# zouyuoz/SVS-UNet-PyTorch

Hardware: AMD Instinct MI355X
Metric: spectrogram-tiles/sec (512x128) U-Net fwd+bwd (L1 train step incl. Adam) (higher is better)
Workload: dtype f32; 1 GPU; train.py L1-loss step, 512x128 tiles, batch 64 per GPU; global_batch=64, parallelism=dp1, mode=train

## Files before the change

### svs_unet_pytorch_amd/csrc/gemm_wgrad.hip

```cpp
#include <stdlib.h>

#include "internal.h"
#include "mfma_split.h"

struct WgradArgs {
  const float* s; long lds; int Hs, Ws, Cs;
  const float* l; long ldl; int Hl, Wl, Cl;
  int B;
  float* slab;
  long pix_per_split;
  int ws_shift, hs_shift;
  int b_shift;
};

template <int T> __device__ __forceinline__ void load_vec(const float* p, float (&f)[T]);
template <> __device__ __forceinline__ void load_vec<4>(const float* p, float (&f)[4]) {
  const f32x4 v = *(const f32x4*)p; f[0] = v[0]; f[1] = v[1]; f[2] = v[2]; f[3] = v[3];
}
template <> __device__ __forceinline__ void load_vec<2>(const float* p, float (&f)[2]) {
  const float2 v = *(const float2*)p; f[0] = v.x; f[1] = v.y;
}
template <int T> __device__ __forceinline__ void store_vec(float* p, const float (&f)[T]);
template <> __device__ __forceinline__ void store_vec<4>(float* p, const float (&f)[4]) { *(f32x4*)p = (f32x4){f[0], f[1], f[2], f[3]}; }
template <> __device__ __forceinline__ void store_vec<2>(float* p, const float (&f)[2]) { *(float2*)p = make_float2(f[0], f[1]); }

template <int BM, int BN, int WM, int WN, bool SKIP = false, bool SPLIT = false, int PF = 1>
__global__ __launch_bounds__(256) void wgrad_gemm_kernel(WgradArgs p) {
  constexpr int TM = BM / WM / 16;
  constexpr int TN = BN / WN / 16;
  constexpr int LDA = BM + 4, LDB = BN + 4;
  constexpr int CA = BM / 4, CB = BN / 4;
  constexpr int RA = (16 * CA + 255) / 256, RB = (16 * CB + 255) / 256;
  static_assert(WM * WN == 4, "4 waves");

  __shared__ __attribute__((aligned(16))) float As[2][16 * LDA];
  __shared__ __attribute__((aligned(16))) float Bs[2][16 * LDB];

  const int t = threadIdx.x;
  const int lane = t & 63, wave = t >> 6;
  const int wm = wave / WN, wn = wave % WN;
  const int lrow = lane & 15, q = lane >> 4;

  const int Ntot = 25 * p.Cl;
  const int cs0 = blockIdx.x * BM;
  const int n0 = blockIdx.y * BN;
  const long P = (long)p.B * p.Hs * p.Ws;
  const long p_begin = (long)blockIdx.z * p.pix_per_split;
  long p_end = p_begin + p.pix_per_split;
  if (p_end > P) p_end = P;

  constexpr unsigned OOB = 0x80000000u;
  int ak[RA], ac[RA]; bool aok[RA];
#pragma unroll
  for (int r = 0; r < RA; ++r) {
    const int idx = t + 256 * r;
    ak[r] = idx / CA; ac[r] = idx % CA; aok[r] = idx < 16 * CA;
  }
  int bk[RB], bc[RB], bkh[RB], bkw[RB], bcl[RB]; bool bok[RB];
#pragma unroll
  for (int r = 0; r < RB; ++r) {
    const int idx = t + 256 * r;
    bk[r] = idx / CB; bc[r] = idx % CB;
    const int n = n0 + bc[r] * 4;
    bok[r] = (idx < 16 * CB) && (n < Ntot);
    const int tap = bok[r] ? n / p.Cl : 0;
    bcl[r] = bok[r] ? n - tap * p.Cl : 0;
    bkh[r] = tap / 5; bkw[r] = tap - bkh[r] * 5;
  }

  int bj[RB], bi[RB]; unsigned bimg[RB];
#pragma unroll
  for (int r = 0; r < RB; ++r) {
    const unsigned pix = (unsigned)(p_begin + bk[r]);
    const unsigned row = pix / (unsigned)p.Ws;
    bj[r] = (int)(pix - row * (unsigned)p.Ws);
    const unsigned img = row / (unsigned)p.Hs;
    bi[r] = (int)(row - img * (unsigned)p.Hs);
    bimg[r] = img * (unsigned)(p.Hl * p.Wl);
  }
  const unsigned img_stride = (unsigned)(p.Hl * p.Wl);
  auto advance = [&]() {
#pragma unroll
    for (int r = 0; r < RB; ++r) {
      unsigned j = (unsigned)bj[r] + 16u, i = (unsigned)bi[r];
      if (p.ws_shift >= 0) { i += j >> p.ws_shift; j &= (unsigned)p.Ws - 1u; }
      else { const unsigned q = j / (unsigned)p.Ws; j -= q * (unsigned)p.Ws; i += q; }
      unsigned nb;
      if (p.hs_shift >= 0) { nb = i >> p.hs_shift; i &= (unsigned)p.Hs - 1u; }
      else { nb = i / (unsigned)p.Hs; i -= nb * (unsigned)p.Hs; }
      bj[r] = (int)j; bi[r] = (int)i; bimg[r] += nb * img_stride;
    }
  };

  unsigned a_voff[RA];
#pragma unroll
  for (int r = 0; r < RA; ++r) a_voff[r] = aok[r] ? (unsigned)(((long)ak[r] * p.lds + cs0 + ac[r] * 4) * 4) : OOB;
  const __amdgpu_buffer_rsrc_t rs = __builtin_amdgcn_make_buffer_rsrc((void*)(p.s + p_begin * p.lds), 0, OOB, 0x00020000);
  const __amdgpu_buffer_rsrc_t rl = __builtin_amdgcn_make_buffer_rsrc((void*)p.l, 0, OOB, 0x00020000);
  const int HsWs = p.Hs * p.Ws, HlWl = p.Hl * p.Wl;
  unsigned a_voff_s[RA], b_voff_s[RB];
  int tap_lo = 0, tap_hi = 0;
  if (SKIP) {
#pragma unroll
    for (int r = 0; r < RA; ++r) a_voff_s[r] = aok[r] ? (unsigned)((((long)ak[r] * HsWs) * p.lds + cs0 + ac[r] * 4) * 4) : OOB;
#pragma unroll
    for (int r = 0; r < RB; ++r)
      b_voff_s[r] = (unsigned)((((long)bk[r] * HlWl + bkh[r] * p.Wl + bkw[r]) * p.ldl + bcl[r]) * 4);
    tap_lo = n0 / p.Cl;
    const int nlast = (n0 + BN - 1 < Ntot - 1) ? n0 + BN - 1 : Ntot - 1;
    tap_hi = nlast / p.Cl;
  }
  const __amdgpu_buffer_rsrc_t rs_all = __builtin_amdgcn_make_buffer_rsrc((void*)p.s, 0, OOB, 0x00020000);
  const __amdgpu_buffer_rsrc_t rl_sh = __builtin_amdgcn_make_buffer_rsrc((void*)(p.l - (2L * p.Wl + 2) * p.ldl), 0, OOB, 0x00020000);
  auto position = [&](int pk, int& i, int& j, int& b0) {
    const int pos = pk >> p.b_shift;
    b0 = pk & (p.B - 1);
    i = pos >> p.ws_shift;
    j = pos & (p.Ws - 1);
  };
  auto first_valid = [&](int pk) -> int {
    if (!SKIP) return pk;
    while (pk < (int)p_end) {
      int i, j, b0;
      position(pk, i, j, b0);
      bool any = false;
      for (int tp = tap_lo; tp <= tap_hi; ++tp) {
        const int kh = tp / 5, kw = tp - kh * 5;
        any = any || ((unsigned)(2 * i - 2 + kh) < (unsigned)p.Hl && (unsigned)(2 * j - 2 + kw) < (unsigned)p.Wl);
      }
      if (any) return pk;
      pk = ((pk >> p.b_shift) + 1) << p.b_shift;
    }
    return (int)p_end;
  };
  f32x4 ra[RA], rb[RB];
  f32x4 ra2[PF == 2 ? RA : 1], rb2[PF == 2 ? RB : 1];
  auto load_tile_skip = [&](int pk, f32x4 (&ra)[RA], f32x4 (&rb)[RB]) __attribute__((always_inline)) {
    int i, j, b0;
    position(pk, i, j, b0);
    const int soff_a = __builtin_amdgcn_readfirstlane((int)((((long)b0 * HsWs + (i * p.Ws + j)) * p.lds) * 4));
    const int soff_b = __builtin_amdgcn_readfirstlane((int)((((long)b0 * HlWl + 2 * i * p.Wl + 2 * j) * p.ldl) * 4));
    const int left = (int)p_end - pk;
#pragma unroll
    for (int r = 0; r < RA; ++r) {
      const unsigned vo = ak[r] < left ? a_voff_s[r] : OOB;
      ra[r] = __builtin_bit_cast(f32x4, __builtin_amdgcn_raw_buffer_load_b128(rs_all, (int)vo, soff_a, 0));
    }
#pragma unroll
    for (int r = 0; r < RB; ++r) {
      const int ih = 2 * i - 2 + bkh[r], iw = 2 * j - 2 + bkw[r];
      const bool ok = bok[r] && bk[r] < left && (unsigned)ih < (unsigned)p.Hl && (unsigned)iw < (unsigned)p.Wl;
      rb[r] = __builtin_bit_cast(f32x4, __builtin_amdgcn_raw_buffer_load_b128(rl_sh, (int)(ok ? b_voff_s[r] : OOB), soff_b, 0));
    }
  };
  auto load_tile = [&](long pk, f32x4 (&ra)[RA], f32x4 (&rb)[RB]) __attribute__((always_inline)) {
    const int soff_a = (int)((pk - p_begin) * p.lds * 4);
    const int left = (int)(p_end - pk);
#pragma unroll
    for (int r = 0; r < RA; ++r) {
      const unsigned vo = ak[r] < left ? a_voff[r] : OOB;
      ra[r] = __builtin_bit_cast(f32x4, __builtin_amdgcn_raw_buffer_load_b128(rs, (int)vo, soff_a, 0));
    }
#pragma unroll
    for (int r = 0; r < RB; ++r) {
      const int ih = 2 * bi[r] - 2 + bkh[r], iw = 2 * bj[r] - 2 + bkw[r];
      const bool ok = bok[r] && bk[r] < left && (unsigned)ih < (unsigned)p.Hl && (unsigned)iw < (unsigned)p.Wl;
      const unsigned vo = ((bimg[r] + (unsigned)(ih * p.Wl + iw)) * (unsigned)p.ldl + (unsigned)bcl[r]) * 4u;
      rb[r] = __builtin_bit_cast(f32x4, __builtin_amdgcn_raw_buffer_load_b128(rl, (int)(ok ? vo : OOB), 0, 0));
    }
    advance();
  };
  auto store_tile = [&](int buf, const f32x4 (&ra)[RA], const f32x4 (&rb)[RB]) __attribute__((always_inline)) {
#pragma unroll
    for (int r = 0; r < RA; ++r)
      if (aok[r]) *(f32x4*)(&As[buf][ak[r] * LDA + ac[r] * 4]) = ra[r];
#pragma unroll
    for (int r = 0; r < RB; ++r)
      if (t + 256 * r < 16 * CB) *(f32x4*)(&Bs[buf][bk[r] * LDB + bc[r] * 4]) = rb[r];
  };

  f32x4 acc[TM][TN];
#pragma unroll
  for (int i = 0; i < TM; ++i)
// ... 36 lines not shown
  if constexpr (PF == 2) {
    int pk1 = first_valid(pk + 16);
    if (pk < (int)p_end) fetch(pk, ra, rb);
    if (pk1 < (int)p_end) fetch(pk1, ra2, rb2);
    if (pk < (int)p_end) store_tile(0, ra, rb);
    __syncthreads();
    while (pk < (int)p_end) {
      int pk2 = first_valid(pk1 + 16);
      if (pk2 < (int)p_end) fetch(pk2, ra, rb);
      multiply(0);
      if (pk1 < (int)p_end) store_tile(1, ra2, rb2);
      __syncthreads();
      pk = pk1; pk1 = pk2;
      if (pk >= (int)p_end) break;
      pk2 = first_valid(pk1 + 16);
      if (pk2 < (int)p_end) fetch(pk2, ra2, rb2);
      multiply(1);
      if (pk1 < (int)p_end) store_tile(0, ra, rb);
      __syncthreads();
      pk = pk1; pk1 = pk2;
    }
  } else {
    if (pk < (int)p_end) {
      fetch(pk, ra, rb);
      store_tile(0, ra, rb);
    }
    __syncthreads();
    for (int it = 0; pk < (int)p_end; ++it) {
      const int buf = it & 1;
      const int pkn = first_valid(pk + 16);
      const bool more = pkn < (int)p_end;
      if (more) fetch(pkn, ra, rb);
      pk = pkn;
      multiply(buf);
      if (more) store_tile(buf ^ 1, ra, rb);
      __syncthreads();
    }
  }

  float* slab = p.slab + (long)blockIdx.z * p.Cs * Ntot;
#pragma unroll
  for (int i = 0; i < TM; ++i)
#pragma unroll
    for (int r = 0; r < 4; ++r) {
      const int cs = cs0 + wm * (TM * 16) + TM * (4 * q + r) + i;
      const int n = n0 + wn * (TN * 16) + TN * lrow;
      if (n < Ntot) {
        float v[TN];
#pragma unroll
        for (int j = 0; j < TN; ++j) v[j] = acc[i][j][r];
        store_vec<TN>(&slab[(long)cs * Ntot + n], v);
      }
    }
}

struct WgWinArgs {
  const float* s; long lds; const float* l; long ldl;
  int B, Hs, Ws, Cs, Hl, Wl, Cl;
  float* slab;
  int ntiles, tiles_per_block;
};

template <int MT>
__global__ __launch_bounds__(256, 2) void wgrad_window_kernel(WgWinArgs p) {
  constexpr int TH = 4, TW = 16, KS = 4 / MT, CSB = 16 * MT;
  constexpr int LS = CSB + 16;
  constexpr int LH = 2 * TH + 3, LW = 2 * TW + 3, LL = 24;
  constexpr int NS = TH * TW * (CSB / 4), NL = LH * LW * 4;
  constexpr int RS = (NS + 255) / 256, RL = (NL + 255) / 256;
  constexpr int KSTEPS = TH * TW / 4 / KS;
  constexpr unsigned OOB = 0x80000000u;
  __shared__ __attribute__((aligned(16))) float Ssm[TH * TW * LS];
  __shared__ __attribute__((aligned(16))) float Lsm[LH * LW * LL];
  const int t = threadIdx.x, lane = t & 63, wave = t >> 6;
  const int lrow = lane & 15, q = lane >> 4;
  const int mt = wave % MT, half = wave / MT;
  const int mchunks = p.Cs / CSB;
  const int m0 = (blockIdx.y % mchunks) * CSB, cl0 = (blockIdx.y / mchunks) * 16;
  const int tiles_w = (p.Ws + TW - 1) / TW, tiles_h = (p.Hs + TH - 1) / TH;
  const int tile_lo = blockIdx.x * p.tiles_per_block;
  const int tile_hi = min(tile_lo + p.tiles_per_block, p.ntiles);

  f32x4 sreg[RS], lreg[RL];
  auto fetch = [&](int tile) {
    const int tw0 = (tile % tiles_w) * TW, th0 = ((tile / tiles_w) % tiles_h) * TH;
    const long b = tile / (tiles_w * tiles_h);
    const __amdgpu_buffer_rsrc_t rs = __builtin_amdgcn_make_buffer_rsrc((void*)(p.s + b * p.Hs * p.Ws * p.lds), 0, OOB, 0x00020000);
    const __amdgpu_buffer_rsrc_t rl = __builtin_amdgcn_make_buffer_rsrc((void*)(p.l + b * p.Hl * p.Wl * p.ldl), 0, OOB, 0x00020000);
#pragma unroll
    for (int r = 0; r < RS; ++r) {
      const int e = t + 256 * r;
      const int c4 = e % (CSB / 4), px = e / (CSB / 4);
      const int sh = th0 + px / TW, sw = tw0 + px % TW;
      const bool ok = e < NS && sh < p.Hs && sw < p.Ws;
      const unsigned vo = ok ? (unsigned)(((sh * p.Ws + sw) * (int)p.lds + m0 + c4 * 4) * 4) : OOB;
      sreg[r] = __builtin_bit_cast(f32x4, __builtin_amdgcn_raw_buffer_load_b128(rs, (int)vo, 0, 0));
    }
#pragma unroll
    for (int r = 0; r < RL; ++r) {
      const int e = t + 256 * r;
      const int c4 = e & 3, px = e >> 2;
      const int ih = 2 * th0 - 2 + px / LW, iw = 2 * tw0 - 2 + px % LW;
      const bool ok = e < NL && (unsigned)ih < (unsigned)p.Hl && (unsigned)iw < (unsigned)p.Wl;
      const unsigned vo = ok ? (unsigned)(((ih * p.Wl + iw) * (int)p.ldl + cl0 + c4 * 4) * 4) : OOB;
      lreg[r] = __builtin_bit_cast(f32x4, __builtin_amdgcn_raw_buffer_load_b128(rl, (int)vo, 0, 0));
    }
  };
  auto stage = [&]() {
#pragma unroll
    for (int r = 0; r < RS; ++r) {
      const int e = t + 256 * r;
      if (e < NS) *(f32x4*)(&Ssm[(e / (CSB / 4)) * LS + (e % (CSB / 4)) * 4]) = sreg[r];
    }
#pragma unroll
    for (int r = 0; r < RL; ++r) {
      const int e = t + 256 * r;
      if (e < NL) *(f32x4*)(&Lsm[(e >> 2) * LL + (e & 3) * 4]) = lreg[r];
    }
  };

  f32x4 acc[25];
#pragma unroll
  for (int i = 0; i < 25; ++i) acc[i] = (f32x4){0.f, 0.f, 0.f, 0.f};
  const float* abase = &Ssm[(half * (TH / KS) * TW + q) * LS + mt * 16 + lrow];
  const float* bbase = &Lsm[(half * (TH / KS) * 2 * LW + 2 * q) * LL + lrow];

  if (tile_lo < tile_hi) fetch(tile_lo);
  for (int tile = tile_lo; tile < tile_hi; ++tile) {
    __syncthreads();
    stage();
    __syncthreads();
    if (tile + 1 < tile_hi) fetch(tile + 1);
#pragma unroll
    for (int ks = 0; ks < KSTEPS; ++ks) {
      const int sh = ks / 4, sg = ks % 4;
      const float a = abase[(sh * TW + sg * 4) * LS];
#pragma unroll
      for (int tap = 0; tap < 25; ++tap) {
        const int kh = tap / 5, kw = tap % 5;
        const float bv = bbase[((2 * sh + kh) * LW + 8 * sg + kw) * LL];
        acc[tap] = __builtin_amdgcn_mfma_f32_16x16x4f32(a, bv, acc[tap], 0, 0, 0);
      }
    }
  }
  const int Ntot = 25 * p.Cl;
  float* slab = p.slab + ((long)blockIdx.x * KS + half) * p.Cs * Ntot;
#pragma unroll
  for (int tap = 0; tap < 25; ++tap)
#pragma unroll
    for (int r = 0; r < 4; ++r)
      slab[(long)(m0 + mt * 16 + 4 * q + r) * Ntot + tap * p.Cl + cl0 + lrow] = acc[tap][r];
}

__global__ __launch_bounds__(256) void wgrad_reduce_kernel(const float* __restrict__ slab, int ksplit, int Cs, int Cl,
                                                           float* __restrict__ dw) {
  __shared__ float tile[25][65];
  const int clt = Cl < 64 ? Cl : 64;
  const int cs = blockIdx.x, cl0 = blockIdx.y * clt;
  const long zstride = (long)Cs * Cl * 25;
  const float* src0 = slab + (long)cs * 25 * Cl + cl0;
  const int q4 = clt >> 2;
  for (int e = threadIdx.x; e < 25 * q4; e += 256) {
    const int tap = e / q4, cl = (e - tap * q4) * 4;
    const float* src = src0 + (long)tap * Cl + cl;
    f32x4 acc = {0.f, 0.f, 0.f, 0.f};
    int z = 0;
    for (; z + 4 <= ksplit; z += 4, src += 4 * zstride) {
      const f32x4 a = *(const f32x4*)src, b = *(const f32x4*)(src + zstride), c = *(const f32x4*)(src + 2 * zstride), d = *(const f32x4*)(src + 3 * zstride);
      acc += a; acc += b; acc += c; acc += d;
    }
    for (; z < ksplit; ++z, src += zstride) acc += *(const f32x4*)src;
    tile[tap][cl] = acc[0]; tile[tap][cl + 1] = acc[1]; tile[tap][cl + 2] = acc[2]; tile[tap][cl + 3] = acc[3];
  }
  __syncthreads();
  float* dst = dw + ((long)cs * Cl + cl0) * 25;
  for (int e = threadIdx.x; e < 25 * clt; e += 256) {
    const int cl = e / 25, tap = e - cl * 25;
    dst[e] = tile[tap][cl];
  }
}

struct WgradTile { int cfg, BM, BN, ksplit; long pps; };
static WgradTile plan_wgrad(int B, int Hs, int Ws, int Cs, int Cl) {
  WgradTile pl{};
  if (Cs % 128 == 0) { pl.cfg = 0; pl.BM = 128; }
  else if (Cs % 64 == 0) { pl.cfg = 1; pl.BM = 64; }
  else { pl.cfg = 2; pl.BM = 32; }
  if (pl.cfg == 0 && ((long)B * Hs * Ws <= 1024 || Cl <= 32)) { pl.cfg = 1; pl.BM = 64; }
  if (svs_tune_on(SVS_TUNE_WGRAD_CFG)) {
    const int c = (int)svs_tune(SVS_TUNE_WGRAD_CFG);
    if (c == 0 && Cs % 128 == 0) { pl.cfg = 0; pl.BM = 128; }
    if (c == 1 && Cs % 64 == 0) { pl.cfg = 1; pl.BM = 64; }
    if (c == 2 && Cs % 32 == 0) { pl.cfg = 2; pl.BM = 32; }
  }
  pl.BN = 128;
  const long P = (long)B * Hs * Ws;
  const long blocks_mn = (long)(Cs / pl.BM) * ((25L * Cl + pl.BN - 1) / pl.BN);
  long ks = (1024 + blocks_mn - 1) / blocks_mn;
  const long cap = P / 128 > 1 ? P / 128 : 1;
  if (ks > cap) ks = cap;
  if (ks > 512) ks = 512;
  if (ks < 1) ks = 1;
  if (svs_tune_on(SVS_TUNE_WGRAD_KSPLIT)) { long f = svs_tune(SVS_TUNE_WGRAD_KSPLIT); if (f >= 1 && f <= cap) ks = f; }
  long pps = (P + ks - 1) / ks;
  pps = (pps + 15) / 16 * 16;
  ks = (P + pps - 1) / pps;
  pl.ksplit = (int)ks;
  pl.pps = pps;
  return pl;
}

#define WG_GROUPS 8

struct WgWinPlan { int eligible, use, MT, gy, gx, tpb, ntiles, nslab; };
static WgWinPlan plan_wgrad_window(int B, int Hs, int Ws, int Cs, int Cl) {
  WgWinPlan w{};
  w.eligible = (Cl == 16 || Cl == 32) && (Cs == 32 || Cs == 64 || Cs == 128);
  w.ntiles = B * ((Hs + 3) / 4) * ((Ws + 15) / 16);
  w.use = w.eligible && w.ntiles >= 1024;
  if (svs_tune_on(SVS_TUNE_WGRAD_WINDOW)) { const int f = (int)svs_tune(SVS_TUNE_WGRAD_WINDOW); w.use = (f == 0) ? 0 : (f == 2) ? w.eligible : w.use; }
  if (!w.eligible) return w;
  w.MT = (Cs % 64 == 0) ? 4 : 2;
  w.gy = (Cs / (16 * w.MT)) * (Cl / 16);
  int gx = 512 / w.gy;
  if (gx > w.ntiles) gx = w.ntiles;
  w.tpb = (w.ntiles + gx - 1) / gx;
  w.gx = (w.ntiles + w.tpb - 1) / w.tpb;
  w.nslab = w.gx * (4 / w.MT);
  return w;
}

struct WgradPlan {
  WgWinPlan win;
  WgradTile tile;
  int WM, WN, pf;
  bool skip, split;
  dim3 grid;
  int nslab;
};
static WgradPlan plan_wgrad_call(int B, int Hs, int Ws, int Cs, int Cl, long lds, int Hl, int Wl, long ldl) {
  WgradPlan p{};
  p.win = plan_wgrad_window(B, Hs, Ws, Cs, Cl);
  p.win.use = p.win.use && (long)Hs * Ws * lds * 4 < (1L << 31) && (long)Hl * Wl * ldl * 4 < (1L << 31);
  if (p.win.use) {
    p.grid = dim3(p.win.gx, p.win.gy);
    p.nslab = p.win.nslab;
    return p;
  }
  p.tile = plan_wgrad(B, Hs, Ws, Cs, Cl);
  p.WM = p.tile.cfg == 0 ? 2 : 1;
  p.WN = 4 / p.WM;
  const bool can_skip = B >= 16 && (B & (B - 1)) == 0 && (Ws & (Ws - 1)) == 0 && (long)B * Hs * Ws * lds * 4 < (1L << 31);
  const long f = svs_tune(SVS_TUNE_WGRAD_SKIP);
  p.skip = f == 0 ? false : f == 2 ? can_skip : can_skip && Ws <= 8;
  p.pf = p.skip && p.tile.cfg <= 1 ? 2 : 1;
  p.split = svs_tune(SVS_TUNE_MFMA_SPLIT) > 0;
  p.grid = dim3((unsigned)(Cs / p.tile.BM), (unsigned)((25 * Cl + p.tile.BN - 1) / p.tile.BN), (unsigned)p.tile.ksplit);
  p.nslab = p.tile.ksplit;
  return p;
}

size_t svs_wgrad_gemm_workspace(int B, int Hs, int Ws, int Cs, int Cl) {
  const WgWinPlan w = plan_wgrad_window(B, Hs, Ws, Cs, Cl);
  int nslab = plan_wgrad(B, Hs, Ws, Cs, Cl).ksplit;
  if (w.eligible && w.nslab > nslab) nslab = w.nslab;
  return ((size_t)nslab + WG_GROUPS) * Cs * 25 * Cl * sizeof(float);
}

static int wgrad_reduce_run(const float* slabs, int nslab, int Cs, int Cl, float* dw, float* tmp, hipStream_t stream) {
  const long n = (long)Cs * 25 * Cl;
  if (nslab > 2 * WG_GROUPS) {
    const int per = (nslab + WG_GROUPS - 1) / WG_GROUPS;
    const int groups = (nslab + per - 1) / per;
    if (int rc = svs_reduce_slabs_run(slabs, nslab, per, groups, n, tmp, stream)) return rc;
    slabs = tmp;
    nslab = groups;
  }
  hipLaunchKernelGGL(wgrad_reduce_kernel, dim3((unsigned)Cs, (unsigned)((Cl + 63) / 64)), dim3(256), 0, stream, slabs, nslab, Cs,
                     Cl, dw);
  SVS_CHECK_LAUNCH("wgrad_reduce");
  return SVS_OK;
}

template <bool SPLIT, int BM, int WM, int WN>
static void launch_wgrad_tile(const WgradArgs& a, const WgradPlan& p, hipStream_t stream) {
  constexpr int PF2 = BM == 32 ? 1 : 2;
  if (!p.skip) hipLaunchKernelGGL((wgrad_gemm_kernel<BM, 128, WM, WN, false, SPLIT>), p.grid, dim3(256), 0, stream, a);
  else if (p.pf == 2) hipLaunchKernelGGL((wgrad_gemm_kernel<BM, 128, WM, WN, true, SPLIT, PF2>), p.grid, dim3(256), 0, stream, a);
  else hipLaunchKernelGGL((wgrad_gemm_kernel<BM, 128, WM, WN, true, SPLIT>), p.grid, dim3(256), 0, stream, a);
}
template <bool SPLIT>
static void launch_wgrad_gemm(const WgradArgs& a, const WgradPlan& p, hipStream_t stream) {
  switch (p.tile.cfg) {
    case 0: launch_wgrad_tile<SPLIT, 128, 2, 2>(a, p, stream); break;
    case 1: launch_wgrad_tile<SPLIT, 64, 1, 4>(a, p, stream); break;
    default: launch_wgrad_tile<SPLIT, 32, 1, 4>(a, p, stream); break;
  }
}

int svs_wgrad_gemm_run(const float* s, long lds, int B, int Hs, int Ws, int Cs, const float* l, long ldl, int Hl,
                       int Wl, int Cl, float* dw, void* ws, size_t ws_bytes, hipStream_t stream, const char* who) {
  SVS_REQUIRE(s && l && dw, "%s: null pointer", who);
  SVS_REQUIRE(Cs >= 32 && Cs % 32 == 0 && Cl >= 16 && Cl % 4 == 0, "%s: unsupported channels Cs=%d Cl=%d", who, Cs, Cl);
  SVS_REQUIRE(Hs == svs_conv_out(Hl) && Ws == svs_conv_out(Wl), "%s: small grid %dx%d does not match %dx%d", who, Hs, Ws, Hl, Wl);
  SVS_REQUIRE(lds >= Cs && lds % 4 == 0 && ldl >= Cl && ldl % 4 == 0, "%s: bad ld", who);
  SVS_REQUIRE(svs_aligned16(s) && svs_aligned16(l) && svs_aligned16(ws), "%s: pointers must be 16-byte aligned", who);
  const size_t need = svs_wgrad_gemm_workspace(B, Hs, Ws, Cs, Cl);
  if (!ws || ws_bytes < need) {
    svs_set_error("%s: workspace too small (%zu < %zu)", who, ws_bytes, need);
    return SVS_ERR_WORKSPACE;
  }
  const WgradPlan p = plan_wgrad_call(B, Hs, Ws, Cs, Cl, lds, Hl, Wl, ldl);
  if (p.win.use) {
    WgWinArgs wa{s, lds, l, ldl, B, Hs, Ws, Cs, Hl, Wl, Cl, (float*)ws, p.win.ntiles, p.win.tpb};
    if (p.win.MT == 4) hipLaunchKernelGGL((wgrad_window_kernel<4>), p.grid, dim3(256), 0, stream, wa);
    else hipLaunchKernelGGL((wgrad_window_kernel<2>), p.grid, dim3(256), 0, stream, wa);
    SVS_CHECK_LAUNCH("wgrad_window");
  } else {
    WgradArgs a{};
    a.s = s; a.lds = lds; a.Hs = Hs; a.Ws = Ws; a.Cs = Cs;
    a.l = l; a.ldl = ldl; a.Hl = Hl; a.Wl = Wl; a.Cl = Cl;
    a.B = B; a.slab = (float*)ws; a.pix_per_split = p.tile.pps;
    auto log2_or_neg = [](int v) { int s = 0; while ((1 << s) < v) ++s; return (1 << s) == v ? s : -1; };
    a.ws_shift = log2_or_neg(Ws); a.hs_shift = log2_or_neg(Hs);
    SVS_REQUIRE((long)B * Hs * Ws < (1L << 31), "%s: pixel count exceeds 2^31", who);
    SVS_REQUIRE((long)B * Hl * Wl * ldl * 4 < (1L << 31) && (long)(p.tile.pps + 16) * lds * 4 < (1L << 31),
                "%s: operand views need 64-bit offsets; split the batch", who);
    if (p.skip) a.b_shift = log2_or_neg(B);
    if (p.split) launch_wgrad_gemm<true>(a, p, stream);
    else launch_wgrad_gemm<false>(a, p, stream);
    SVS_CHECK_LAUNCH("wgrad_gemm");
  }
  if (svs_tune_flag(SVS_TUNE_SKIP_REDUCE)) return SVS_OK;
  return wgrad_reduce_run((const float*)ws, p.nslab, Cs, Cl, dw, (float*)ws + (size_t)p.nslab * Cs * 25 * Cl, stream);
}

int svs_wgrad_gemm_describe(int B, int Hs, int Ws, int Cs, int Cl, char* buf, size_t n) {
  const WgradPlan p = plan_wgrad_call(B, Hs, Ws, Cs, Cl, Cs, 2 * Hs, 2 * Ws, Cl);
  if (p.win.use) snprintf(buf, n, "wgrad_window_kernel<%d>", p.win.MT);
  else snprintf(buf, n, "wgrad_gemm_kernel<%d, %d, %d, %d, %s, %s, %d>", p.tile.BM, p.tile.BN, p.WM, p.WN, p.skip ? "true" : "false",
                p.split ? "true" : "false", p.pf);
  return p.nslab;
}
```

### svs_unet_pytorch_amd/csrc/internal.h

```cpp
#pragma once
#include "common.h"

enum { SVS_MODE_GATHER = 0, SVS_MODE_PARITY = 1 };

int svs_conv_gemm_run(int mode, const float* x, long ldx, int B, int H, int W, int C, const float* wp,
                      const float* bias, const float* scale, const float* shift, float slope, float* y, long ldy,
                      int Ho, int Wo, int N, int accumulate, void* ws, size_t ws_bytes, hipStream_t stream,
                      const char* who, float* stats = nullptr, int stats_cap = 0, int* stats_nblk = nullptr);
int svs_bn_finalize_run(const void* partial, int nblk, long P, int C, float eps, float momentum, float* running_mean,
                        float* running_var, long long* nbt, float* save_mean, float* save_invstd, hipStream_t stream);
int svs_bn_fin_act_apply_run(const void* partial, int rows, const float* raw, long ldr, long P, int C, long pixels_per_sample,
                             const float* gamma, const float* beta, float eps, float momentum, float* running_mean,
                             float* running_var, long long* nbt, float* save_mean, float* save_invstd, float slope,
                             const float* drop, float* y, long ldy, hipStream_t stream);
struct SvsSumJobs { int njobs; const float* partial[12]; int nblk[12]; int C[12]; float* out[12]; };
int svs_channel_sum_finalize_multi_run(const SvsSumJobs& jobs, hipStream_t stream);
size_t svs_bn_partial_floats(long P, int C);
int svs_bn_partial_rows(long P, int C);
size_t svs_conv_gemm_workspace(int mode, int B, int H, int W, int C, int Ho, int Wo, int N);

int svs_wgrad_gemm_run(const float* s, long lds, int B, int Hs, int Ws, int Cs, const float* l, long ldl, int Hl,
                       int Wl, int Cl, float* dw, void* ws, size_t ws_bytes, hipStream_t stream, const char* who);
size_t svs_wgrad_gemm_workspace(int B, int Hs, int Ws, int Cs, int Cl);

int svs_conv_c1_run(const float* x, int B, int H, int W, const float* w, const float* bias, const float* scale,
                    const float* shift, float slope, float* y, long ldy, int N, int accumulate, hipStream_t stream,
                    const char* who, long half = 0);
int svs_deconv_to1_run(const float* x, long ldx, int B, int H, int W, int C, const float* w, const float* bias,
                       float* y, int Ho, int Wo, int apply_sigmoid, hipStream_t stream, const char* who, long half = 0);
int svs_wgrad_c1_run(const float* s, long lds, int B, int Hs, int Ws, int Cs, const float* l, int Hl, int Wl,
                     float* dw, void* ws, size_t ws_bytes, hipStream_t stream, const char* who, long half = 0);
size_t svs_wgrad_c1_workspace(int B, int Hs, int Ws, int Cs);

int svs_channel_sum_run(const float* x, long ldx, long P, int C, float* out, void* ws, size_t ws_bytes, hipStream_t stream);
int svs_sum_run(const float* x, long n, float* out, void* ws, size_t ws_bytes, hipStream_t stream);
int svs_sigmoid_bwd_run(const float* mask, const float* dmask, long n, float* d_logit, hipStream_t stream);

int svs_reduce_slabs_run(const float* slab, int nslab, int per, int groups, long n, float* out, hipStream_t stream);

struct SvsPackJob { const float* w; float* wp; int N, C, kind, first_block; };
struct SvsPackJobs { SvsPackJob j[20]; int n; };
int svs_pack_all_run(SvsPackJobs& jobs, hipStream_t stream);

int svs_bn_bwd_run(const float* dy, long lddy, const float* raw, long ldr, long P, int C, long pixels_per_sample,
                   const float* gamma, const float* beta, const float* save_mean, const float* save_invstd, float slope,
                   const float* drop, float* d_raw, float* dgamma, float* dbeta, float* dbias, void* ws, size_t ws_bytes,
                   hipStream_t stream, float* dbias_partial = nullptr, SvsSumJobs* defer = nullptr);

int svs_fft_twiddles(int n, hipStream_t stream, const float2** out);
int svs_fft_hann(int n, hipStream_t stream, const float** out);

int svs_conv_gemm_describe(int mode, int B, int H, int W, int C, int Ho, int Wo, int N, long ldx, char* buf, size_t n);
int svs_wgrad_gemm_describe(int B, int Hs, int Ws, int Cs, int Cl, char* buf, size_t n);
int svs_conv_bf16_describe(int mode, int B, int H, int W, int C, int Ho, int Wo, int N, char* buf, size_t n);
```

### svs_unet_pytorch_amd/csrc/special.hip

```cpp
#include "internal.h"

struct C1Args {
  const float* x; int B, H, W;
  const float* w;
  const float* bias; const float* scale; const float* shift; float slope;
  float* y; long ldy; int Ho, Wo; int accumulate;
  long half;
};

__device__ __forceinline__ long chan_off(long pix, long ld, int sub, int subs_per_half, long half) {
  return pix * ld + (half ? (sub >= subs_per_half ? half + (sub - subs_per_half) * 4 : sub * 4) : sub * 4);
}

template <int COUT>
__global__ __launch_bounds__(256) void conv_c1_kernel(C1Args p) {
  constexpr int G = COUT / 4;
  constexpr int LD = COUT + 4;
  __shared__ __attribute__((aligned(16))) float tile[256 * LD];
  const float* __restrict__ w = p.w;
  const long P = (long)p.B * p.Ho * p.Wo;
  const long pix0 = (long)blockIdx.x * 256;
  const long pix = pix0 + threadIdx.x;
  if (pix < P) {
    const unsigned upix = (unsigned)pix, utmp = upix / (unsigned)p.Wo;
// ... 288 lines not shown
  constexpr int G = CS / 4;
  constexpr int PL = 256 / G;
  __shared__ float red[4][25 * CS];
  const int t = threadIdx.x;
  const int cg = t % G, pl = t / G;
  const long P = (long)p.B * p.Hs * p.Ws;
  const long p0 = (long)blockIdx.x * p.pix_per_block;
  long p1 = p0 + p.pix_per_block;
  if (p1 > P) p1 = P;
  f32x4 acc[25];
#pragma unroll
  for (int k = 0; k < 25; ++k) acc[k] = (f32x4){0.f, 0.f, 0.f, 0.f};
  for (long pix = p0 + pl; pix < p1; pix += PL) {
    const int j = (int)(pix % p.Ws);
    const long tmp = pix / p.Ws;
    const int i = (int)(tmp % p.Hs);
    const long b = tmp / p.Hs;
    const f32x4 s4 = *(const f32x4*)(p.s + chan_off(pix, p.lds, cg, G / 2, p.half));
    const float* img = p.l + b * p.Hl * p.Wl;
    constexpr int NM = (25 + G - 1) / G;
    float mine[NM];
#pragma unroll
    for (int m = 0; m < NM; ++m) {
      const int tap = cg + G * m;
      const int kh = tap / 5, kw = tap - kh * 5;
      const int ih = 2 * i - 2 + kh, iw = 2 * j - 2 + kw;
      float lv = 0.f;
      if (tap < 25 && (unsigned)ih < (unsigned)p.Hl && (unsigned)iw < (unsigned)p.Wl) lv = img[(long)ih * p.Wl + iw];
      mine[m] = lv;
    }
    const int group = (t & 63) & ~(G - 1);
#pragma unroll
    for (int tap = 0; tap < 25; ++tap) {
      const float lv = __shfl(mine[tap / G], group | (tap % G), 64);
      acc[tap] += s4 * lv;
    }
  }
#pragma unroll
  for (int k = 0; k < 25; ++k)
#pragma unroll
    for (int c = 0; c < 4; ++c) {
      float v = acc[k][c];
#pragma unroll
      for (int s = G; s < 64; s <<= 1) v += __shfl_xor(v, s, 64);
      acc[k][c] = v;
    }
  const int lane = t & 63, wave = t >> 6;
  if (lane < G) {
#pragma unroll
    for (int k = 0; k < 25; ++k)
#pragma unroll
      for (int c = 0; c < 4; ++c) red[wave][(lane * 4 + c) * 25 + k] = acc[k][c];
  }
  __syncthreads();
  float* out = p.slab + (long)blockIdx.x * (25 * CS);
  for (int i = t; i < 25 * CS; i += 256) out[i] = (red[0][i] + red[1][i]) + (red[2][i] + red[3][i]);
}

template <int CS>
__global__ __launch_bounds__(256) void wgrad_c1_mfma_kernel(WgC1Args p, int ntiles, int tiles_per_wave) {
  constexpr int TH = 4, TW = 16, MT = CS / 16;
  constexpr int LS = (CS == 32) ? 48 : 16;
  constexpr int LH = 2 * TH + 3, LW = 2 * TW + 3, LWP = LW + 1;
  constexpr int NSP = TH * TW * (CS / 4) / 64;
  constexpr int NLP = (LH * LW + 63) / 64;
  __shared__ __attribute__((aligned(16))) float Ssm[4][TH * TW * LS];
  __shared__ float Lsm[4][LH * LWP];
  const int t = threadIdx.x, lane = t & 63, wave = t >> 6;
  const int lrow = lane & 15, q = lane >> 4;
  float* const sS = Ssm[wave];
  float* const sL = Lsm[wave];
  const int tiles_w = (p.Ws + TW - 1) / TW, tiles_h = (p.Hs + TH - 1) / TH;
  const int gw = blockIdx.x * 4 + wave;
  const int tile_lo = gw * tiles_per_wave;
  const int tile_hi = min(tile_lo + tiles_per_wave, ntiles);

  f32x4 sreg[NSP];
  float lreg[NLP];
  auto fetch = [&](int tile) {
    const int tw0 = (tile % tiles_w) * TW, th0 = ((tile / tiles_w) % tiles_h) * TH;
    const long b = tile / (tiles_w * tiles_h);
#pragma unroll
    for (int r = 0; r < NSP; ++r) {
      const int e = lane + 64 * r;
      const int c4 = e % (CS / 4), px = e / (CS / 4);
      const int sh = th0 + px / TW, sw = tw0 + px % TW;
      f32x4 v = {0.f, 0.f, 0.f, 0.f};
      if (sh < p.Hs && sw < p.Ws) v = *(const f32x4*)(p.s + chan_off((b * p.Hs + sh) * p.Ws + sw, p.lds, c4, CS / 8, p.half));
      sreg[r] = v;
    }
    const float* img = p.l + b * p.Hl * p.Wl;
#pragma unroll
    for (int r = 0; r < NLP; ++r) {
      const int e = lane + 64 * r;
      const int wr = e / LW, wc = e % LW;
      const int ih = 2 * th0 - 2 + wr, iw = 2 * tw0 - 2 + wc;
      float v = 0.f;
      if (e < LH * LW && (unsigned)ih < (unsigned)p.Hl && (unsigned)iw < (unsigned)p.Wl) v = img[(long)ih * p.Wl + iw];
      lreg[r] = v;
    }
  };
  auto stage = [&]() {
#pragma unroll
    for (int r = 0; r < NSP; ++r) {
      const int e = lane + 64 * r;
      *(f32x4*)(&sS[(e / (CS / 4)) * LS + (e % (CS / 4)) * 4]) = sreg[r];
    }
#pragma unroll
    for (int r = 0; r < NLP; ++r) {
      const int e = lane + 64 * r;
      if (e < LH * LW) sL[(e / LW) * LWP + e % LW] = lreg[r];
    }
  };
  f32x4 acc[MT][2];
#pragma unroll
  for (int i = 0; i < MT; ++i) { acc[i][0] = (f32x4){0.f, 0.f, 0.f, 0.f}; acc[i][1] = acc[i][0]; }
  int boff[2];
#pragma unroll
  for (int nt = 0; nt < 2; ++nt) {
    const int tap = min(nt * 16 + lrow, 24);
    boff[nt] = (tap / 5) * LWP + tap % 5 + 2 * q;
  }
  if (tile_lo < tile_hi) fetch(tile_lo);
  for (int tile = tile_lo; tile < tile_hi; ++tile) {
    stage();
    if (tile + 1 < tile_hi) fetch(tile + 1);
#pragma unroll
    for (int ks = 0; ks < TH * TW / 4; ++ks) {
      const int sh = ks / 4, sg = ks % 4;
      float bv[2];
#pragma unroll
      for (int nt = 0; nt < 2; ++nt) bv[nt] = sL[boff[nt] + 2 * sh * LWP + 8 * sg];
#pragma unroll
      for (int i = 0; i < MT; ++i) {
        const float a = sS[(sh * TW + sg * 4 + q) * LS + i * 16 + lrow];
#pragma unroll
        for (int nt = 0; nt < 2; ++nt) acc[i][nt] = __builtin_amdgcn_mfma_f32_16x16x4f32(a, bv[nt], acc[i][nt], 0, 0, 0);
      }
    }
  }
  float* out = p.slab + (long)gw * (25 * CS);
#pragma unroll
  for (int i = 0; i < MT; ++i)
#pragma unroll
    for (int nt = 0; nt < 2; ++nt) {
      const int tap = nt * 16 + lrow;
      if (tap < 25) {
#pragma unroll
        for (int r = 0; r < 4; ++r) out[(i * 16 + 4 * q + r) * 25 + tap] = acc[i][nt][r];
      }
    }
}

__global__ __launch_bounds__(256) void reduce_slabs_kernel(const float* __restrict__ slab, int nslab, int per, long n,
                                                           float* __restrict__ out) {
  const long i = ((long)blockIdx.x * 256 + threadIdx.x) * 4;
  if (i >= n) return;
  const int z0 = blockIdx.y * per;
  int z1 = z0 + per;
  if (z1 > nslab) z1 = nslab;
  const float* src = slab + (long)z0 * n + i;
  f32x4 s = {0.f, 0.f, 0.f, 0.f};
  int z = z0;
  for (; z + 4 <= z1; z += 4, src += 4 * n) {
    const f32x4 a = *(const f32x4*)src, b = *(const f32x4*)(src + n), c = *(const f32x4*)(src + 2 * n), d = *(const f32x4*)(src + 3 * n);
    s += a; s += b; s += c; s += d;
  }
  for (; z < z1; ++z, src += n) s += *(const f32x4*)src;
  *(f32x4*)(out + (long)blockIdx.y * n + i) = s;
}

int svs_reduce_slabs_run(const float* slab, int nslab, int per, int groups, long n, float* out, hipStream_t stream) {
  hipLaunchKernelGGL(reduce_slabs_kernel, dim3((unsigned)((n / 4 + 255) / 256), (unsigned)groups), dim3(256), 0, stream, slab, nslab, per, n, out);
  SVS_CHECK_LAUNCH("reduce_slabs");
  return SVS_OK;
}

#define C1_GROUPS 32

static int wgrad_c1_blocks(long P) {
  long nb = (P + 2047) / 2048;
  if (nb > 1024) nb = 1024;
  if (nb < 1) nb = 1;
  return (int)nb;
}

size_t svs_wgrad_c1_workspace(int B, int Hs, int Ws, int Cs) {
  (void)B; (void)Hs; (void)Ws;
  return (size_t)(1024 + C1_GROUPS) * 25 * Cs * sizeof(float);
}

int svs_wgrad_c1_run(const float* s, long lds, int B, int Hs, int Ws, int Cs, const float* l, int Hl, int Wl,
                     float* dw, void* ws, size_t ws_bytes, hipStream_t stream, const char* who, long half) {
  SVS_REQUIRE(s && l && dw, "%s: null pointer", who);
  SVS_REQUIRE(Cs == 16 || Cs == 32, "%s: supports Cs=16/32, got %d", who, Cs);
  SVS_REQUIRE(Hs == svs_conv_out(Hl) && Ws == svs_conv_out(Wl), "%s: grid mismatch", who);
  SVS_REQUIRE(lds >= (half ? Cs / 2 : Cs) && lds % 4 == 0 && svs_aligned16(s), "%s: bad view", who);
  const long P = (long)B * Hs * Ws;
  const int nb = wgrad_c1_blocks(P);
  const size_t need = svs_wgrad_c1_workspace(B, Hs, Ws, Cs);
  if (!ws || ws_bytes < need) {
    svs_set_error("%s: workspace too small (%zu < %zu)", who, ws_bytes, need);
    return SVS_ERR_WORKSPACE;
  }
  WgC1Args a{s, lds, B, Hs, Ws, l, Hl, Wl, (float*)ws, (P + nb - 1) / nb, half};
  int nslab = nb;
  const int ntiles = B * ((Hs + 3) / 4) * ((Ws + 15) / 16);
  if (ntiles >= 256) {
    int waves = ntiles < 1024 ? ntiles : 1024;
    waves = (waves + 3) / 4 * 4;
    if (waves > 1024) waves = 1024;
    const int tpw = (ntiles + waves - 1) / waves;
    waves = ((ntiles + tpw - 1) / tpw + 3) / 4 * 4;
    nslab = waves;
    if (Cs == 16) hipLaunchKernelGGL(wgrad_c1_mfma_kernel<16>, dim3(waves / 4), dim3(256), 0, stream, a, ntiles, tpw);
    else hipLaunchKernelGGL(wgrad_c1_mfma_kernel<32>, dim3(waves / 4), dim3(256), 0, stream, a, ntiles, tpw);
  } else if (Cs == 16) hipLaunchKernelGGL(wgrad_c1_kernel<16>, dim3(nb), dim3(256), 0, stream, a);
  else hipLaunchKernelGGL(wgrad_c1_kernel<32>, dim3(nb), dim3(256), 0, stream, a);
  SVS_CHECK_LAUNCH("wgrad_c1");
  const long n = 25L * Cs;
  float* tmp = (float*)ws + (size_t)nslab * n;
  const int groups = nslab < C1_GROUPS ? nslab : C1_GROUPS;
  const int per = (nslab + groups - 1) / groups;
  const unsigned gx = (unsigned)((n / 4 + 255) / 256);
  hipLaunchKernelGGL(reduce_slabs_kernel, dim3(gx, (unsigned)groups), dim3(256), 0, stream, (const float*)ws, nslab, per, n, tmp);
  SVS_CHECK_LAUNCH("reduce_slabs");
  hipLaunchKernelGGL(reduce_slabs_kernel, dim3(gx, 1), dim3(256), 0, stream, (const float*)tmp, groups, groups, n, dw);
  SVS_CHECK_LAUNCH("reduce_slabs");
  return SVS_OK;
}
```

Before: 19040 tiles/s.

## Fuse two-pass slab reductions into a single-kernel grouped slab sum

Replaces the two-kernel split-K slab reduction (a grouped partial-sum kernel, then a final reduce through a temporary buffer) with one kernel. Each block has its thread groups sum slab ranges, parks the partials in LDS and combines them in-block, so the intermediate global buffer and one launch go away for both the wgrad GEMM and the c1 wgrad paths. It also changes the GEMM LDS padding from +4 to either no padding or +8, depending on the per-wave tile count. The risks are fewer blocks feeding the reduction, which lowers parallelism for large slab counts, and possible bank conflicts from the new pitch.

```diff
diff --git a/svs_unet_pytorch_amd/csrc/gemm_wgrad.hip b/svs_unet_pytorch_amd/csrc/gemm_wgrad.hip
--- a/svs_unet_pytorch_amd/csrc/gemm_wgrad.hip
+++ b/svs_unet_pytorch_amd/csrc/gemm_wgrad.hip
@@ -13,6 +13,72 @@
   int b_shift;
 };
 
+#define SLAB_SUM_LDS (25 * 65)
+__device__ __forceinline__ f32x4 slab_chain(const float* src, int z, int z1, long zstride) {
+  f32x4 acc = {0.f, 0.f, 0.f, 0.f};
+  for (; z + 4 <= z1; z += 4, src += 4 * zstride) {
+    const f32x4 a = *(const f32x4*)src, b = *(const f32x4*)(src + zstride), c = *(const f32x4*)(src + 2 * zstride), d = *(const f32x4*)(src + 3 * zstride);
+    acc += a; acc += b; acc += c; acc += d;
+  }
+  for (; z < z1; ++z, src += zstride) acc += *(const f32x4*)src;
+  return acc;
+}
+__device__ __forceinline__ void slab_sum_block(const SvsSlabSum& s, int rb, float* lds) {
+  const int t = threadIdx.x;
+  const long zstride = (long)s.Cs * s.row;
+  if (s.groups > 0) {
+    const int seg = 256 / s.gcap, q4 = s.row >> 2;
+    const int nseg = (q4 + seg - 1) / seg;
+    const int cs = rb / nseg, c0 = (rb - cs * nseg) * seg;
+    const int g = t / seg, col = c0 + (t - g * seg);
+    f32x4 sum = {0.f, 0.f, 0.f, 0.f};
+    if (g < s.groups && col < q4) {
+      const int z0 = g * s.per;
+      const int z1 = z0 + s.per < s.nslab ? z0 + s.per : s.nslab;
+      if (z0 < z1) sum = slab_chain(s.slabs + z0 * zstride + (long)cs * s.row + col * 4, z0, z1, zstride);
+    }
+    f32x4* park = (f32x4*)lds;
+    park[t] = sum;
+    __syncthreads();
+    if (t < seg && col < q4) {
+      f32x4 acc = {0.f, 0.f, 0.f, 0.f};
+      for (int k = 0; k < s.groups; ++k) acc += park[k * seg + t];
+      if (s.Cl > 0) {
+        const int tap = (col * 4) / s.Cl, cl = col * 4 - tap * s.Cl;
+        float* dst = s.dw + ((long)cs * s.Cl + cl) * 25 + tap;
+        dst[0] = acc[0]; dst[25] = acc[1]; dst[50] = acc[2]; dst[75] = acc[3];
+      } else {
+        *(f32x4*)(s.dw + (long)cs * s.row + col * 4) = acc;
+      }
+    }
+    return;
+  }
+  float (*tile)[65] = (float (*)[65])lds;
+  const int Cl = s.Cl;
+  const int cchunks = (Cl + 63) / 64;
+  const int cs = rb / cchunks, cl0 = (rb - cs * cchunks) * 64;
+  const int clt = Cl - cl0 < 64 ? Cl - cl0 : 64;
+  const float* src0 = s.slabs + (long)cs * 25 * Cl + cl0;
+  const int q4 = clt >> 2;
+  for (int e = t; e < 25 * q4; e += 256) {
+    const int tap = e / q4, cl = (e - tap * q4) * 4;
+    const f32x4 acc = slab_chain(src0 + (long)tap * Cl + cl, 0, s.nslab, zstride);
+    tile[tap][cl] = acc[0]; tile[tap][cl + 1] = acc[1]; tile[tap][cl + 2] = acc[2]; tile[tap][cl + 3] = acc[3];
+  }
+  __syncthreads();
+  float* dst = s.dw + ((long)cs * Cl + cl0) * 25;
+  for (int e = t; e < 25 * clt; e += 256) {
+    const int cl = e / 25, tap = e - cl * 25;
+    dst[e] = tile[tap][cl];
+  }
+}
+__global__ __launch_bounds__(256) void slab_sum_kernel(SvsSlabSum s) {
+  __shared__ __attribute__((aligned(16))) float lds[SLAB_SUM_LDS];
+  slab_sum_block(s, blockIdx.x, lds);
+}
+
+constexpr int wgrad_pitch(int width, int T) { return T == 4 ? width : width + 8; }
+
 template <int T> __device__ __forceinline__ void load_vec(const float* p, float (&f)[T]);
 template <> __device__ __forceinline__ void load_vec<4>(const float* p, float (&f)[4]) {
   const f32x4 v = *(const f32x4*)p; f[0] = v[0]; f[1] = v[1]; f[2] = v[2]; f[3] = v[3];
@@ -28,7 +94,8 @@
 __global__ __launch_bounds__(256) void wgrad_gemm_kernel(WgradArgs p) {
   constexpr int TM = BM / WM / 16;
   constexpr int TN = BN / WN / 16;
-  constexpr int LDA = BM + 4, LDB = BN + 4;
+  constexpr int LDA = wgrad_pitch(BM, TM), LDB = wgrad_pitch(BN, TN);
+  static_assert(BM % 16 == 0 && BN % 16 == 0 && (TM == 2 || TM == 4) && (TN == 2 || TN == 4), "wgrad_pitch");
   constexpr int CA = BM / 4, CB = BN / 4;
   constexpr int RA = (16 * CA + 255) / 256, RB = (16 * CB + 255) / 256;
   static_assert(WM * WN == 4, "4 waves");
@@ -371,34 +438,6 @@
       slab[(long)(m0 + mt * 16 + 4 * q + r) * Ntot + tap * p.Cl + cl0 + lrow] = acc[tap][r];
 }
 
-__global__ __launch_bounds__(256) void wgrad_reduce_kernel(const float* __restrict__ slab, int ksplit, int Cs, int Cl,
-                                                           float* __restrict__ dw) {
-  __shared__ float tile[25][65];
-  const int clt = Cl < 64 ? Cl : 64;
-  const int cs = blockIdx.x, cl0 = blockIdx.y * clt;
-  const long zstride = (long)Cs * Cl * 25;
-  const float* src0 = slab + (long)cs * 25 * Cl + cl0;
-  const int q4 = clt >> 2;
-  for (int e = threadIdx.x; e < 25 * q4; e += 256) {
-    const int tap = e / q4, cl = (e - tap * q4) * 4;
-    const float* src = src0 + (long)tap * Cl + cl;
-    f32x4 acc = {0.f, 0.f, 0.f, 0.f};
-    int z = 0;
-    for (; z + 4 <= ksplit; z += 4, src += 4 * zstride) {
-      const f32x4 a = *(const f32x4*)src, b = *(const f32x4*)(src + zstride), c = *(const f32x4*)(src + 2 * zstride), d = *(const f32x4*)(src + 3 * zstride);
-      acc += a; acc += b; acc += c; acc += d;
-    }
-    for (; z < ksplit; ++z, src += zstride) acc += *(const f32x4*)src;
-    tile[tap][cl] = acc[0]; tile[tap][cl + 1] = acc[1]; tile[tap][cl + 2] = acc[2]; tile[tap][cl + 3] = acc[3];
-  }
-  __syncthreads();
-  float* dst = dw + ((long)cs * Cl + cl0) * 25;
-  for (int e = threadIdx.x; e < 25 * clt; e += 256) {
-    const int cl = e / 25, tap = e - cl * 25;
-    dst[e] = tile[tap][cl];
-  }
-}
-
 struct WgradTile { int cfg, BM, BN, ksplit; long pps; };
 static WgradTile plan_wgrad(int B, int Hs, int Ws, int Cs, int Cl) {
   WgradTile pl{};
@@ -483,21 +522,29 @@
   const WgWinPlan w = plan_wgrad_window(B, Hs, Ws, Cs, Cl);
   int nslab = plan_wgrad(B, Hs, Ws, Cs, Cl).ksplit;
   if (w.eligible && w.nslab > nslab) nslab = w.nslab;
-  return ((size_t)nslab + WG_GROUPS) * Cs * 25 * Cl * sizeof(float);
-}
-
-static int wgrad_reduce_run(const float* slabs, int nslab, int Cs, int Cl, float* dw, float* tmp, hipStream_t stream) {
-  const long n = (long)Cs * 25 * Cl;
-  if (nslab > 2 * WG_GROUPS) {
-    const int per = (nslab + WG_GROUPS - 1) / WG_GROUPS;
-    const int groups = (nslab + per - 1) / per;
-    if (int rc = svs_reduce_slabs_run(slabs, nslab, per, groups, n, tmp, stream)) return rc;
-    slabs = tmp;
-    nslab = groups;
-  }
-  hipLaunchKernelGGL(wgrad_reduce_kernel, dim3((unsigned)Cs, (unsigned)((Cl + 63) / 64)), dim3(256), 0, stream, slabs, nslab, Cs,
-                     Cl, dw);
-  SVS_CHECK_LAUNCH("wgrad_reduce");
+  return (size_t)nslab * Cs * 25 * Cl * sizeof(float);
+}
+
+SvsSlabSum svs_slab_sum_plan(const float* slabs, int nslab, int Cs, int Cl, int row, float* dw, int gcap, bool always_groups) {
+  SvsSlabSum s{};
+  s.slabs = slabs; s.dw = dw; s.nslab = nslab; s.gcap = gcap; s.Cs = Cs; s.Cl = Cl; s.row = row;
+  if (always_groups) {
+    s.groups = nslab < gcap ? nslab : gcap;
+    s.per = (nslab + s.groups - 1) / s.groups;
+  } else if (nslab > 2 * gcap) {
+    s.per = (nslab + gcap - 1) / gcap;
+    s.groups = (nslab + s.per - 1) / s.per;
+  }
+  if (s.groups > 0) s.R = Cs * ((row / 4 + 256 / gcap - 1) / (256 / gcap));
+  else s.R = Cs * ((Cl + 63) / 64);
+  return s;
+}
+int svs_slab_sum_run(const SvsSlabSum& s, hipStream_t stream) {
+  if (!s.R) return SVS_OK;
+  SVS_REQUIRE(s.row % 4 == 0 && (s.groups > 0 || s.Cl > 0) && (s.groups == 0 || (s.gcap > 0 && 256 % s.gcap == 0 && s.groups <= s.gcap)),
+              "slab_sum: bad plan");
+  hipLaunchKernelGGL(slab_sum_kernel, dim3((unsigned)s.R), dim3(256), 0, stream, s);
+  SVS_CHECK_LAUNCH("slab_sum");
   return SVS_OK;
 }
 
@@ -551,7 +598,7 @@
     SVS_CHECK_LAUNCH("wgrad_gemm");
   }
   if (svs_tune_flag(SVS_TUNE_SKIP_REDUCE)) return SVS_OK;
-  return wgrad_reduce_run((const float*)ws, p.nslab, Cs, Cl, dw, (float*)ws + (size_t)p.nslab * Cs * 25 * Cl, stream);
+  return svs_slab_sum_run(svs_slab_sum_plan((const float*)ws, p.nslab, Cs, Cl, 25 * Cl, dw, WG_GROUPS, false), stream);
 }
 
 int svs_wgrad_gemm_describe(int B, int Hs, int Ws, int Cs, int Cl, char* buf, size_t n) {
diff --git a/svs_unet_pytorch_amd/csrc/internal.h b/svs_unet_pytorch_amd/csrc/internal.h
--- a/svs_unet_pytorch_amd/csrc/internal.h
+++ b/svs_unet_pytorch_amd/csrc/internal.h
@@ -19,6 +19,15 @@
 int svs_bn_partial_rows(long P, int C);
 size_t svs_conv_gemm_workspace(int mode, int B, int H, int W, int C, int Ho, int Wo, int N);
 
+struct SvsSlabSum {
+  const float* slabs; float* dw;
+  int nslab, per, groups, gcap;
+  int Cs, Cl, row;
+  int R;
+};
+SvsSlabSum svs_slab_sum_plan(const float* slabs, int nslab, int Cs, int Cl, int row, float* dw, int gcap, bool always_groups);
+int svs_slab_sum_run(const SvsSlabSum& s, hipStream_t stream);
+
 int svs_wgrad_gemm_run(const float* s, long lds, int B, int Hs, int Ws, int Cs, const float* l, long ldl, int Hl,
                        int Wl, int Cl, float* dw, void* ws, size_t ws_bytes, hipStream_t stream, const char* who);
 size_t svs_wgrad_gemm_workspace(int B, int Hs, int Ws, int Cs, int Cl);
@@ -36,8 +45,6 @@
 int svs_sum_run(const float* x, long n, float* out, void* ws, size_t ws_bytes, hipStream_t stream);
 int svs_sigmoid_bwd_run(const float* mask, const float* dmask, long n, float* d_logit, hipStream_t stream);
 
-int svs_reduce_slabs_run(const float* slab, int nslab, int per, int groups, long n, float* out, hipStream_t stream);
-
 struct SvsPackJob { const float* w; float* wp; int N, C, kind, first_block; };
 struct SvsPackJobs { SvsPackJob j[20]; int n; };
 int svs_pack_all_run(SvsPackJobs& jobs, hipStream_t stream);
diff --git a/svs_unet_pytorch_amd/csrc/special.hip b/svs_unet_pytorch_amd/csrc/special.hip
--- a/svs_unet_pytorch_amd/csrc/special.hip
+++ b/svs_unet_pytorch_amd/csrc/special.hip
@@ -464,30 +464,6 @@
     }
 }
 
-__global__ __launch_bounds__(256) void reduce_slabs_kernel(const float* __restrict__ slab, int nslab, int per, long n,
-                                                           float* __restrict__ out) {
-  const long i = ((long)blockIdx.x * 256 + threadIdx.x) * 4;
-  if (i >= n) return;
-  const int z0 = blockIdx.y * per;
-  int z1 = z0 + per;
-  if (z1 > nslab) z1 = nslab;
-  const float* src = slab + (long)z0 * n + i;
-  f32x4 s = {0.f, 0.f, 0.f, 0.f};
-  int z = z0;
-  for (; z + 4 <= z1; z += 4, src += 4 * n) {
-    const f32x4 a = *(const f32x4*)src, b = *(const f32x4*)(src + n), c = *(const f32x4*)(src + 2 * n), d = *(const f32x4*)(src + 3 * n);
-    s += a; s += b; s += c; s += d;
-  }
-  for (; z < z1; ++z, src += n) s += *(const f32x4*)src;
-  *(f32x4*)(out + (long)blockIdx.y * n + i) = s;
-}
-
-int svs_reduce_slabs_run(const float* slab, int nslab, int per, int groups, long n, float* out, hipStream_t stream) {
-  hipLaunchKernelGGL(reduce_slabs_kernel, dim3((unsigned)((n / 4 + 255) / 256), (unsigned)groups), dim3(256), 0, stream, slab, nslab, per, n, out);
-  SVS_CHECK_LAUNCH("reduce_slabs");
-  return SVS_OK;
-}
-
 #define C1_GROUPS 32
 
 static int wgrad_c1_blocks(long P) {
@@ -499,7 +475,7 @@
 
 size_t svs_wgrad_c1_workspace(int B, int Hs, int Ws, int Cs) {
   (void)B; (void)Hs; (void)Ws;
-  return (size_t)(1024 + C1_GROUPS) * 25 * Cs * sizeof(float);
+  return (size_t)1024 * 25 * Cs * sizeof(float);
 }
 
 int svs_wgrad_c1_run(const float* s, long lds, int B, int Hs, int Ws, int Cs, const float* l, int Hl, int Wl,
@@ -530,14 +506,5 @@
   } else if (Cs == 16) hipLaunchKernelGGL(wgrad_c1_kernel<16>, dim3(nb), dim3(256), 0, stream, a);
   else hipLaunchKernelGGL(wgrad_c1_kernel<32>, dim3(nb), dim3(256), 0, stream, a);
   SVS_CHECK_LAUNCH("wgrad_c1");
-  const long n = 25L * Cs;
-  float* tmp = (float*)ws + (size_t)nslab * n;
-  const int groups = nslab < C1_GROUPS ? nslab : C1_GROUPS;
-  const int per = (nslab + groups - 1) / groups;
-  const unsigned gx = (unsigned)((n / 4 + 255) / 256);
-  hipLaunchKernelGGL(reduce_slabs_kernel, dim3(gx, (unsigned)groups), dim3(256), 0, stream, (const float*)ws, nslab, per, n, tmp);
-  SVS_CHECK_LAUNCH("reduce_slabs");
-  hipLaunchKernelGGL(reduce_slabs_kernel, dim3(gx, 1), dim3(256), 0, stream, (const float*)tmp, groups, groups, n, dw);
-  SVS_CHECK_LAUNCH("reduce_slabs");
-  return SVS_OK;
-}
+  return svs_slab_sum_run(svs_slab_sum_plan((const float*)ws, nslab, 1, 0, 25 * Cs, dw, C1_GROUPS, true), stream);
+}
```

Result: no change. 18940 tiles/s (-0.6%).
